# z430/keyword-spotting

Measured on AMD Instinct MI355X. Metric: 1s 16kHz clips/sec end-to-end (wav->label), higher is better.
Workload: dtype f32

## Files before the change

keyword-spotting_amd/csrc/kws_dscnn.hip:

```cpp
#include <array>
#include <utility>

#include "kws_dscnn_stages.h"

namespace kws {
namespace {

#ifndef KWS_X_DSCNN_STAMP_TID
#define KWS_X_DSCNN_STAMP_TID 0
#endif

__device__ __forceinline__ DscnnWeights weights_for_this_clip() {
#if defined(__HIP_DEVICE_COMPILE__)
    using KArg = const __attribute__((address_space(4))) DscnnWeights*;
    KArg p = (KArg)__builtin_amdgcn_kernarg_segment_ptr();
    asm volatile("" : "+s"(p));
    return *p;
#else
    return DscnnWeights{};
#endif
}

using FwdKernelFn = void (*)(DscnnWeights, const float*, int, float*, int32_t*, float*, unsigned long long*, const int*, StreamPush);
struct FwdKernelArgs {
// ... 3 lines not shown
    float* logits;
    int32_t* label;
    float* act;
    unsigned long long* stamps;
    const int* ring_hops;
    StreamPush sp;
};

__device__ __forceinline__ ScanWindows scan_windows_now() {
#if defined(__HIP_DEVICE_COMPILE__)
    using KArg = const __attribute__((address_space(4))) FwdKernelArgs*;
    KArg p = (KArg)__builtin_amdgcn_kernarg_segment_ptr();
    asm volatile("" : "+s"(p));
    return p->sp.scan;
#else
    return ScanWindows{};
#endif
}

template <bool SCAN>
__device__ __forceinline__ const float* clip_features(const float* __restrict__ feat, int clip, const ScanWindows& sw) {
    if constexpr (SCAN) {
        unsigned rec = __umulhi((unsigned)clip, sw.wpr_recip), win = (unsigned)clip - rec * sw.wpr;
        if (win >= sw.wpr) {
            win -= sw.wpr;
            ++rec;
        }
        return feat + (size_t)rec * sw.row_floats + (size_t)win * sw.win_floats;
    } else {
        return feat + (size_t)clip * (IN_T * IN_F);
    }
}

template <bool PAIR, bool SCAN = false>
__device__ __forceinline__ void stage_features_persist(float* lds, const float* __restrict__ feat, int clip, int tid,
                                                       const ScanWindows& sw = ScanWindows{}) {
    constexpr int ST = STAGE_WAVES * 64;
    constexpr int FV = (IN_T * IN_F + ST - 1) / ST;
    static_assert(2 * STAGE_WAVES == NW, "each staging wavefront zeroes the maximum slot of one other wavefront");
    const int lane = tid & 63, wv = tid >> 6;
    const float* f = clip_features<SCAN>(feat, clip, sw);
    float fv[FV];
#pragma unroll
    for (int k = 0; k < FV; ++k) {
        const int i = tid + k * ST;
        fv[k] = i < IN_T * IN_F ? f[i] : 0.f;
    }
    float* featp = lds + OFF_FEAT_P;
    for (int i = tid; i < FEAT_H * FEAT_W; i += ST) {
        const int r = i / FEAT_W - 2, c = i % FEAT_W - 2;
        if (!((unsigned)r < (unsigned)IN_T && (unsigned)c < (unsigned)IN_F)) featp[i] = 0.f;
    }
#pragma unroll
    for (int k = 0; k < FV; ++k) {
        const int i = tid + k * ST;
        if (i < IN_T * IN_F) featp[(i / IN_F + 2) * FEAT_W + (i % IN_F) + 2] = fv[k];
    }
    if constexpr (PAIR) {
        float m = 0.f;
#pragma unroll
        for (int k = 0; k < FV; ++k) m = fmaxf(m, fabsf(fv[k]));
        publish_wave_max(lds, 0, wv, lane, m);
        if (lane == 63) lds[OFF_WMAX + wv + STAGE_WAVES] = 0.f;
    }
}

__device__ __forceinline__ void pool_fc_wave(const DscnnWeights& w, const float* lds, int lane, int clip, float* __restrict__ logits,
                                             int32_t* __restrict__ label, float* __restrict__ a_pool) {
    const int C = w.num_classes;
    float4 fcw[CH / 4];
    float fcb = 0.f;
    const float4* wr = reinterpret_cast<const float4*>(w.fc_w + (lane < C ? lane : 0) * CH);
#pragma unroll
    for (int c = 0; c < CH / 4; ++c) fcw[c] = wr[c];
    if (lane < C) fcb = w.fc_b[lane];
    const float ring_b = w.pw_b[3 * CH + lane];
    constexpr float RING_N = 55.f * 11.f - 53.f * 9.f;
    float s = 0.f;
#pragma unroll
    for (int k = 0; k < NW; ++k) s += lds[OFF_POOLBUF_P + k * CH + lane];
    s = fmaf(RING_N, relu(ring_b), s) * (1.0f / (55.f * 11.f));
    if (a_pool) a_pool[lane] = s;
    float acc = fcb;
#pragma unroll
    for (int c = 0; c < CH / 4; ++c) {
        const float4 a4 = fcw[c];
        acc = fmaf(a4.x, __builtin_bit_cast(float, __builtin_amdgcn_readlane(__builtin_bit_cast(int, s), 4 * c + 0)), acc);
        acc = fmaf(a4.y, __builtin_bit_cast(float, __builtin_amdgcn_readlane(__builtin_bit_cast(int, s), 4 * c + 1)), acc);
        acc = fmaf(a4.z, __builtin_bit_cast(float, __builtin_amdgcn_readlane(__builtin_bit_cast(int, s), 4 * c + 2)), acc);
        acc = fmaf(a4.w, __builtin_bit_cast(float, __builtin_amdgcn_readlane(__builtin_bit_cast(int, s), 4 * c + 3)), acc);
    }
    if (lane < C) logits[(size_t)clip * C + lane] = acc;
    const int idx = wave_argmax_first(lane < C ? acc : -INFINITY, lane, C);
    if (label && lane == 0) label[clip] = idx;
}

// ... 5 lines not shown
                                                           unsigned long long* __restrict__ stamps_arg,
                                                           const int* __restrict__ ring_hops, StreamPush sp) {
    static_assert(!STREAM || (MODE >= 4 && !DIAG && !PRECONV), "the fused push exists for the product paths only");
    static_assert(!PERSIST || ((MODE == 4 || MODE == 5) && !PRECONV && !STREAM), "persistent workgroups: batched product paths only");
    static_assert(!SCAN || ((MODE == 4 || MODE == 5) && !DIAG && !PRECONV && !STREAM && !CLUSTER), "strided windows: batched product paths only");
    constexpr bool PAIR = MODE == 5;
    constexpr int NP = PAIR ? 2 : 3;
    BlockTables t1_pre{};
    static_assert(!CLUSTER || STREAM, "time-tile clusters exist for the streaming push only");
    float* const act = DIAG ? act_arg : nullptr;
    unsigned long long* const stamps = DIAG ? stamps_arg : nullptr;
    extern __shared__ __attribute__((aligned(16))) float lds[];
    constexpr bool MFMA = MODE != 0;
    const int tid_k = threadIdx.x;
    const int lane_k = tid_k & 63, wv_k = tid_k >> 6;

    const int cl_n = CLUSTER ? sp.cluster : 1;
    int clip = CLUSTER ? (int)blockIdx.x / cl_n : (int)blockIdx.x;
    const int cl_tile = CLUSTER ? (int)blockIdx.x - clip * cl_n : 0;
    if (clip >= B) return;
    const int j0 = Blk<4>::H * cl_tile / cl_n, j1 = Blk<4>::H * (cl_tile + 1) / cl_n;
    auto rows = [&](int lo, int hi, int H, int W) { return PosRange{(lo < 0 ? 0 : lo) * W, (hi > H ? H : hi) * W}; };
    const PosRange rg4 = rows(j0, j1, Blk<4>::H, Blk<4>::W), rg3 = rows(j0 - 2, j1, Blk<3>::H, Blk<3>::W),
                   rg2 = rows(j0 - 4, j1, Blk<2>::H, Blk<2>::W), rg1 = rows(j0 - 6, j1, Blk<1>::H, Blk<1>::W),
                   rg0 = rows(j0 - 7, j1 + 1, C1_H, C1_W);
    int n_stamp = 0;
    auto stamp = [&]() {
        if (stamps && tid_k == KWS_X_DSCNN_STAMP_TID) stamps[(size_t)clip * KWS_DSCNN_STAMPS + n_stamp] = __builtin_amdgcn_s_memtime();
        ++n_stamp;
    };

    constexpr bool SPLIT = MODE >= 4;
    constexpr bool UT = PERSIST && PAIR;
    BlockTables t1p{};
    uintx4 c1p[PERSIST ? 7 : 1][NP];
    int prev_clip = -1;
    float* a_prev = nullptr;
    if ((MODE == 4 || MODE == 5) && !CLUSTER && tid_k == 0) lds[OFF_ARRIVE] = 0.f;
    if constexpr (PERSIST) {
        fetch_block_tables(w_arg, 1, tid_k, t1p);
        if (wv_k < STAGE_WAVES) stage_features_persist<PAIR, SCAN>(lds, feat, clip, tid_k, sp.scan);
        load_conv1_frags(w_arg, wv_k, lane_k, c1p);
        __syncthreads();
    }
    for (;;) {
    auto weights_now = [&]() -> DscnnWeights { return PERSIST ? weights_for_this_clip() : w_arg; };
    const DscnnWeights w = weights_now();
    int tid = tid_k;
    if constexpr (PERSIST) {
        int wv_l = __builtin_amdgcn_readfirstlane(wv_k), lane_l = lane_k;
        asm volatile("" : "+s"(wv_l), "+v"(lane_l));
        tid = (wv_l << 6) | (lane_l & 63);
    }
    const int lane = tid & 63, wv = tid >> 6;
    if constexpr (PERSIST) n_stamp = 0;
    if (stamps && tid == KWS_X_DSCNN_STAMP_TID) stamps[(size_t)clip * KWS_DSCNN_STAMPS + KWS_DSCNN_STAMPS - 2] = __builtin_amdgcn_s_memrealtime();
    stamp();

    PwOperands<MODE> wa;
    UnitDesc ud{};
    int hops_before = 0;
    int kx = 0, ky[5] = {0, 0, 0, 0, 0}, sg[5] = {0, 0, 0, 0, 0};
    if constexpr (PERSIST) {
        if constexpr (PAIR) {
            const float mxf = read_stage_max(lds, 0, 1);
            kx = pow2_exp_for(mxf);
            const float bz0 = (w.c1_abs * mxf + w.c1_bmax) * 1.001f;
            cap_units(kx, sg[0], w.k_c1, bz0);
            const float by1 = (w.dw_abs[0] * bz0 + w.dw_bmax[0]) * 1.001f;
            ky[1] = pow2_exp_for(by1);
            cap_units(ky[1], sg[1], w.k_pw[0], (w.pw_abs[0] * by1 + w.pw_bmax[0]) * 1.001f);
            store_block_tables(lds, 1, tid, t1p, pow2f(ky[1]), pow2f(sg[1]), pow2f(ky[1] - sg[0]));
            conv1_build_windows(lds, tid, pow2f(kx), OFF_FEAT_P);
            __syncthreads();
        } else {
            store_block_tables(lds, 1, tid, t1p);
        }
        stamp();
        conv1_phase_split<false, NP>(w, lds, tid, c1p, rg0, pow2f(kx), pow2f(sg[0]), OFF_FEAT_P);
        if (wv == NW - 1 && prev_clip >= 0) {
            pool_fc_wave(w, lds, lane, prev_clip, logits, label, a_prev);
            if (stamps && lane == 0) stamps[(size_t)prev_clip * KWS_DSCNN_STAMPS + 13] = __builtin_amdgcn_s_memtime();
        }
        if constexpr (UT) load_unit_desc(w, 1, wv < Leftover<1>::TILE ? wv : Leftover<1>::TILE, lane, ud);
        load_afrag(w, 1, wv >= 4 ? wv - 4 : 0, lane, wa.ring[0]);
    } else if constexpr (PRECONV) {
        static_assert(!PRECONV || MODE >= 4, "the pre-convolved entry exists for the product (split) path only");
        const float* z = feat + (size_t)clip * (CH * P0);
        fetch_block_tables(w, 1, tid, t1_pre);
        float zmax = 0.f;
        for (int i = tid; i < CH * P0; i += NT) {
            const float v = z[i];
            lds[OFF_Z0 + pidx(i / P0, i % P0, P0 + 2)] = v;
            zmax = fmaxf(zmax, v);
        }
        if (tid < CH) {
            lds[OFF_Z0 + pidx(tid, P0, P0 + 2)] = 0.f;
            lds[OFF_Z0 + pidx(tid, P0 + 1, P0 + 2)] = 0.f;
        }
        if constexpr (PAIR)
            publish_wave_max(lds, 1, wv, lane, zmax);
        else
            store_block_tables(lds, 1, tid, t1_pre);
        if constexpr (Leftover<1>::HAS && (MODE == 4 || MODE == 5) && !CLUSTER)
            load_afrag(w, 1, wv >= 4 ? wv - 4 : 0, lane, wa.ring[0]);
        else
            load_block_head(w, 1, lane, wa);
        stamp();
    } else {
    float* featp = lds + OFF_FEAT;
    const float* f = clip_features<SCAN>(feat, clip, sp.scan);
    constexpr int FV = (IN_T * IN_F + NT - 1) / NT;
// ... 95 lines not shown
    } else {
        conv1_phase<MFMA>(w, lds, tid, a1);
    }
    }
    stamp();
    const DscnnWeights w1 = weights_now();
    __syncthreads();
    stamp();
    float* a = act ? act + (size_t)clip * KWS_ACT_FLOATS_PER_CLIP : nullptr;
    if (a) {
        const float u = PAIR ? pow2f(-sg[0]) : 1.f;
        for (int i = tid; i < CH * P0; i += NT) a[i] = lds[OFF_Z0 + pidx(i / P0, i % P0, P0 + 2)] * u;
        a += CH * P0;
    }
    PairCtx pc;
    if constexpr (PAIR && PRECONV) {
        const float mz0 = read_stage_max(lds, 1, 1);
        const float by1 = (w1.dw_abs[0] * mz0 + w1.dw_bmax[0]) * 1.001f;
        ky[1] = pow2_exp_for(by1);
        cap_units(ky[1], sg[1], w1.k_pw[0], (w1.pw_abs[0] * by1 + w1.pw_bmax[0]) * 1.001f);
        store_block_tables(lds, 1, tid, t1_pre, pow2f(ky[1]), pow2f(sg[1]), pow2f(ky[1]));
        __syncthreads();
    }
    if constexpr (PAIR) {
        const float mz = read_stage_max(lds, 1, 1) * pow2f(-sg[0]);
        const float bz = (w1.pw_abs[0] * ((w1.dw_abs[0] * mz + w1.dw_bmax[0]) * 1.001f) + w1.pw_bmax[0]) * 1.001f;
        const float by = (w1.dw_abs[1] * bz + w1.dw_bmax[1]) * 1.001f;
        ky[2] = pow2_exp_for(by);
        cap_units(ky[2], sg[2], w1.k_pw[1], (w1.pw_abs[1] * by + w1.pw_bmax[1]) * 1.001f);
        pc.s_dww = pow2f(ky[2] - sg[1]);
        pc.s_dwb = pow2f(ky[2]);
        pc.s_pwb = pow2f(sg[2]);
    }
    block_phase<1, MODE, CLUSTER, UT>(w1, lds, tid, wa, ud, nullptr, rg1, pc);
    stamp();
    const DscnnWeights w2 = weights_now();
    __syncthreads();
    stamp();
    if (a) {
        const float u = PAIR ? pow2f(-sg[1]) : 1.f;
        for (int i = tid; i < CH * Blk<1>::POUT; i += NT)
            a[i] = lds[OFF_Z1 + pidx(i / Blk<1>::POUT, i % Blk<1>::POUT, Blk<1>::SOUT)] * u;
        a += CH * Blk<1>::POUT;
    }
    if constexpr (PAIR) {
        const float mz = fmaxf(read_stage_max(lds, 2, 1) * pow2f(-sg[1]), w2.pw_bmax[0]);
        const float bz = (w2.pw_abs[1] * ((w2.dw_abs[1] * mz + w2.dw_bmax[1]) * 1.001f) + w2.pw_bmax[1]) * 1.001f;
        const float by = (w2.dw_abs[2] * bz + w2.dw_bmax[2]) * 1.001f;
        ky[3] = pow2_exp_for(by);
        cap_units(ky[3], sg[3], w2.k_pw[2], (w2.pw_abs[2] * by + w2.pw_bmax[2]) * 1.001f);
        pc.s_dww = pow2f(ky[3] - sg[2]);
        pc.s_dwb = pow2f(ky[3]);
        pc.s_pwb = pow2f(sg[3]);
    }
    block_phase<2, MODE, CLUSTER, UT>(w2, lds, tid, wa, ud, nullptr, rg2, pc);
    stamp();
    const DscnnWeights w3 = weights_now();
    __syncthreads();
    stamp();
    if (a) {
        const float u = PAIR ? pow2f(-sg[2]) : 1.f;
        for (int i = tid; i < CH * Blk<2>::POUT; i += NT)
            a[i] = lds[OFF_Z2 + pidx(i / Blk<2>::POUT, i % Blk<2>::POUT, Blk<2>::SOUT)] * u;
        a += CH * Blk<2>::POUT;
    }
    if constexpr (PAIR) {
        const float mz = fmaxf(read_stage_max(lds, 0, 1) * pow2f(-sg[2]), w3.pw_bmax[1]);
        const float bz = (w3.pw_abs[2] * ((w3.dw_abs[2] * mz + w3.dw_bmax[2]) * 1.001f) + w3.pw_bmax[2]) * 1.001f;
        const float by = (w3.dw_abs[3] * bz + w3.dw_bmax[3]) * 1.001f;
        ky[4] = pow2_exp_for(by);
        cap_units(ky[4], sg[4], w3.k_pw[3], (w3.pw_abs[3] * by + w3.pw_bmax[3]) * 1.001f);
        pc.s_dww = pow2f(ky[4] - sg[3]);
        pc.s_dwb = pow2f(ky[4]);
        pc.s_pwb = pow2f(sg[4]);
    }
    block_phase<3, MODE, CLUSTER, UT>(w3, lds, tid, wa, ud, nullptr, rg3, pc);
    stamp();
    const DscnnWeights w4 = weights_now();
    __syncthreads();
    stamp();
    if (a) {
        const float u = PAIR ? pow2f(-sg[3]) : 1.f;
        for (int i = tid; i < CH * Blk<3>::POUT; i += NT)
            a[i] = lds[OFF_Z3 + pidx(i / Blk<3>::POUT, i % Blk<3>::POUT, Blk<3>::SOUT)] * u;
        a += CH * Blk<3>::POUT;
    }
    if constexpr (PAIR) {
        pc.inv_out = pow2f(-sg[4]);
    }
    block_phase<4, MODE, CLUSTER, UT>(w4, lds, tid, wa, ud, a ? a + CH : nullptr, rg4, pc,
                                      PERSIST ? OFF_POOLBUF_P : OFF_POOLBUF);
    stamp();
    if constexpr (PERSIST) {
        const int next = clip + (int)gridDim.x;
        __builtin_amdgcn_sched_barrier(0);
        const ScanWindows sw_next = SCAN ? scan_windows_now() : ScanWindows{};
        if (wv < STAGE_WAVES && next < B) stage_features_persist<PAIR, SCAN>(lds, feat, next, tid, sw_next);
        stamp();
        load_conv1_frags(w4, wv, lane, c1p);
        __syncthreads();
        stamp();
        if (stamps && tid == KWS_X_DSCNN_STAMP_TID) stamps[(size_t)clip * KWS_DSCNN_STAMPS + KWS_DSCNN_STAMPS - 1] = __builtin_amdgcn_s_memrealtime();
        prev_clip = clip;
        a_prev = a;
        clip = next;
        if (clip >= B) break;
        continue;
    }
    const int C = w4.num_classes;
    float4 fcw[CH / 4];
    float fcb = 0.f, ring_b = 0.f;
    if (wv == 0 && lane < C) {
        const float4* wr = reinterpret_cast<const float4*>(w4.fc_w + lane * CH);
#pragma unroll
        for (int c = 0; c < CH / 4; ++c) fcw[c] = wr[c];
        fcb = w4.fc_b[lane];
    }
    if (tid < CH) ring_b = w4.pw_b[3 * CH + tid];
    __syncthreads();
    stamp();

    float* pooled = lds + OFF_POOLED;
    constexpr float RING_N = 55.f * 11.f - 53.f * 9.f;
    bool run_fc = true;
    if constexpr (CLUSTER) {
        float* part = sp.cl_part + ((size_t)clip * cl_n + cl_tile) * CH;
        if (tid < CH) {
            float s = 0.f;
#pragma unroll
            for (int k = 0; k < NW; ++k) s += lds[OFF_POOLBUF + k * CH + tid];
// ... 182 lines not shown
```

keyword-spotting_amd/csrc/kws_dscnn_geom.h:

```cpp
#pragma once
#include "kws_internal.h"

namespace kws {
namespace {

#ifndef KWS_DSCNN_WAVES
#define KWS_DSCNN_WAVES 8
#endif
constexpr int NW = KWS_DSCNN_WAVES;
constexpr int NT = NW * 64;
constexpr int TW = 30;

constexpr int P0 = C1_H * C1_W;
constexpr int FEAT_H = 103, FEAT_W = 14;
constexpr int OFF_Z3 = 0, OFF_Z2 = 22976, OFF_Z1 = 0, OFF_Z0 = 9152, OFF_FEAT = 18304;
constexpr int OFF_DWTAB = 38784;
constexpr int OFF_PWB = OFF_DWTAB + 2 * 768;
constexpr int OFF_POOLED = OFF_PWB + 2 * 64;
constexpr int OFF_POOLBUF = OFF_DWTAB;
constexpr int OFF_WMAX = OFF_POOLED + 64 + 8;
constexpr int OFF_ARRIVE = OFF_WMAX + 3 * NW;
constexpr int LDS_FLOATS = 40960;
static_assert(OFF_ARRIVE + 1 <= LDS_FLOATS, "LDS overflow");
static_assert(NW * 64 <= 768, "pool scratch must fit one depthwise buffer");
static_assert(OFF_FEAT + FEAT_H * FEAT_W <= OFF_Z2, "feature pad overlaps Z2");
static_assert(CH * 12 <= 2 * NT, "table staging assumes at most two elements per thread");

__host__ __device__ __forceinline__ constexpr int pidx(int c, int p, int S) { return (c >> 1) * 2 * S + 2 * p + (c & 1); }

template <int N>
struct Blk {
    static constexpr int H = 45 + 2 * N, W = 1 + 2 * N;
    static constexpr bool RING = N > 1;
    static constexpr int HI = RING ? H - 2 : H, WI = RING ? W - 2 : W;
    static constexpr int PIN = HI * WI, SIN = PIN + 2;
    static constexpr int POUT = H * W, SOUT = POUT + 2;
    static constexpr int OFF_IN = N == 1 ? OFF_Z0 : N == 2 ? OFF_Z1 : N == 3 ? OFF_Z2 : OFF_Z3;
    static constexpr int OFF_OUT = N == 1 ? OFF_Z1 : N == 2 ? OFF_Z2 : OFF_Z3;
    static constexpr int TILES = (POUT + TW - 1) / TW;
    static constexpr int BUF = (N - 1) & 1;
};

#ifndef KWS_DSCNN_KSPLIT_LEFTOVER
#define KWS_DSCNN_KSPLIT_LEFTOVER 1
#endif
template <int N>
struct Leftover {
    static constexpr bool HAS = KWS_DSCNN_KSPLIT_LEFTOVER && (N == 1 || N == 2);
    static constexpr int TILE = N == 1 ? 4 : 8;
    static constexpr int P0T = TILE * TW;
    static constexpr int NP = HAS ? Blk<N>::POUT - P0T : 1;
    static constexpr int WAVE0 = N == 1 ? 4 : 0;
    static constexpr int OFF_PART = N == 1 ? OFF_Z2 : OFF_Z0;
    static constexpr int CSTRIDE = CH + 4;
    static constexpr int PART = NP * CSTRIDE;
};
static_assert(Blk<1>::TILES == 5 && Blk<2>::TILES == 9, "the leftover tiles are the fifth of block 1 and the ninth of block 2");
static_assert(4 * Leftover<1>::PART <= 38784 - OFF_Z2 && OFF_Z0 + 4 * Leftover<2>::PART <= OFF_FEAT, "partial sums fit their dead planes");
static_assert(Leftover<1>::OFF_PART % 4 == 0 && Leftover<2>::OFF_PART % 4 == 0 && Leftover<1>::CSTRIDE % 4 == 0, "partial sums move as float4s");

constexpr int OFF_FEAT_P = OFF_Z2;
constexpr int OFF_POOLBUF_P = OFF_FEAT_P + 1456;
constexpr int STAGE_WAVES = 4;
static_assert(OFF_FEAT_P >= OFF_Z3 + Blk<3>::SOUT * CH, "the next clip's features must not overlap block 4's input");
static_assert(OFF_FEAT_P + FEAT_H * FEAT_W <= OFF_POOLBUF_P && OFF_POOLBUF_P % 4 == 0, "features and pool partials are disjoint");
static_assert(OFF_POOLBUF_P + NW * CH <= OFF_Z2 + Blk<2>::SOUT * CH && OFF_Z2 + Blk<2>::SOUT * CH <= OFF_DWTAB,
              "pool partials stay inside the Z2 plane, clear of the table buffers the next clip's block 1 rewrites");

}
}
```

keyword-spotting_amd/csrc/kws_dscnn_stages.h:

```cpp
#pragma once
#include <type_traits>

#include "kws_dscnn_geom.h"
#include "kws_dscnn_units.h"
#include "kws_mfcc_dev.h"
#include "kws_split_mfma.h"

namespace kws {
namespace {

template <bool TO_MFMA = false>
__device__ __forceinline__ float stencil3x3(float w0, float w1, float w2, float w3, float w4, float w5, float w6,
                                            float w7, float w8, float b, float up, float mid, float dn, float mask_l,
                                            float mask_r) {
    float c, to_right, to_left;
    asm("v_mul_f32 %1, %3, %13\n\t"
        "v_mul_f32 %2, %5, %13\n\t"
        "v_fma_f32 %0, %4, %13, %12\n\t"
        "v_fmac_f32 %1, %6, %14\n\t"
        "v_fmac_f32 %2, %8, %14\n\t"
        "v_fmac_f32 %0, %7, %14\n\t"
        "v_fmac_f32 %1, %9, %15\n\t"
        "v_fmac_f32 %2, %11, %15\n\t"
        "v_fmac_f32 %0, %10, %15\n\t"
// ... 272 lines not shown
            if (kb + 3 < 7) gather(kb + 3, y[nxt]);
            __builtin_amdgcn_sched_barrier(0);
            product(5);
        }
        if (DUAL && kb + 2 < 7) {
            load_other(kb + 2);
            __builtin_amdgcn_sched_barrier(0);
        }
    }
    acc += acc2;
    occ += occ2;
    if (pos < p_hi) {
#pragma unroll
        for (int r = 0; r < 16; r += 2) {
            const int co = ct * 32 + row_of(r, half);
            const float v0 = relu(fmaf(w.c1_b[co], sig0, acc[r])), v1 = relu(fmaf(w.c1_b[co + 1], sig0, acc[r + 1]));
            *reinterpret_cast<float2*>(z0 + pidx(co, pos, P0 + 2)) = make_float2(v0, v1);
            if constexpr (PAIR) mx = fmaxf(mx, fmaxf(v0, v1));
            if (DUAL) {
                const int oo = (ct ^ 1) * 32 + row_of(r, half);
                const float u0 = relu(fmaf(w.c1_b[oo], sig0, occ[r])), u1 = relu(fmaf(w.c1_b[oo + 1], sig0, occ[r + 1]));
                *reinterpret_cast<float2*>(z0 + pidx(oo, pos, P0 + 2)) = make_float2(u0, u1);
                if constexpr (PAIR) mx = fmaxf(mx, fmaxf(u0, u1));
            }
        }
    }
}

constexpr int C1W_ROWS = FEAT_H;
constexpr int OFF_C1W8 = OFF_Z1;
constexpr int OFF_C1P2 = OFF_C1W8 + 2 * C1W_ROWS * 3 * 4;
static_assert(OFF_C1P2 + 2 * C1W_ROWS * 3 <= OFF_Z0, "conv1's operand windows live where block 1's output goes later");
static_assert(2 * (C1_W - 1) + 9 < FEAT_W && 2 * (C1_H - 1) + 9 < FEAT_H, "window reach inside the padded map");

__device__ __forceinline__ void conv1_build_windows(float* lds, int tid, float sx, int off_feat = OFF_FEAT) {
    const float* featp = lds + off_feat;
    uint32_t* w8 = reinterpret_cast<uint32_t*>(lds + OFF_C1W8);
    uint32_t* p2 = reinterpret_cast<uint32_t*>(lds + OFF_C1P2);
    for (int i = tid; i < C1W_ROWS * 3; i += NT) {
        const float* src = featp + (i / 3) * FEAT_W + 2 * (i % 3);
        const float y[8] = {src[0], src[1], src[2], src[3], src[4], src[5], src[6], src[7]};
        uintx4 hi, lo;
        split_pair8(y, sx, hi, lo);
        *reinterpret_cast<uintx4*>(w8 + i * 4) = hi;
        *reinterpret_cast<uintx4*>(w8 + (C1W_ROWS * 3 + i) * 4) = lo;
        uint32_t h, l;
        split_pair2(src[8], src[9], sx, h, l);
        p2[i] = h;
        p2[C1W_ROWS * 3 + i] = l;
    }
}

template <bool DUAL>
__device__ __forceinline__ void conv1_unit_pairwin(const DscnnWeights& w, const float* lds, float* z0, int ptile, int ct, int lane,
                                                   const uintx4 (&c1f)[7][2], int p_lo, int p_hi, float sig0, float& mx) {
    const int half = lane >> 5, col = lane & 31;
    const int pos = p_lo + ptile * 32 + col;
    const int posc = pos < p_hi ? pos : p_hi - 1;
    const int oh = posc / C1_W, ow = posc % C1_W;
    const int wi = (2 * oh + 5 * half) * 3 + ow;
    const uintx4* w8 = reinterpret_cast<const uintx4*>(lds + OFF_C1W8) + wi;
    const uint32_t* p2 = reinterpret_cast<const uint32_t*>(lds + OFF_C1P2) + wi;
    const floatx16 zero = {0, 0, 0, 0, 0, 0, 0, 0, 0, 0, 0, 0, 0, 0, 0, 0};
    floatx16 acc = zero, acc2 = zero, occ = zero, occ2 = zero;
    const uintx4* osrc = reinterpret_cast<const uintx4*>(w.c1_pair) + (size_t)(ct ^ 1) * (7 * 2 * 64) + lane;
    uintx4 of[DUAL ? 7 : 1][2];
    if (DUAL) {
#pragma unroll
        for (int kb = 0; kb < 7; ++kb) {
            of[kb][0] = osrc[(kb * 2 + 0) * 64];
            of[kb][1] = osrc[(kb * 2 + 1) * 64];
        }
    }
    float4 cb[4], ob[DUAL ? 4 : 1];
#pragma unroll
    for (int q = 0; q < 4; ++q) {
        cb[q] = *reinterpret_cast<const float4*>(w.c1_b + ct * 32 + 8 * q + 4 * half);
        if (DUAL) ob[DUAL ? q : 0] = *reinterpret_cast<const float4*>(w.c1_b + (ct ^ 1) * 32 + 8 * q + 4 * half);
    }
    uintx4 bq[3][2];
    auto b_load = [&](int kb, uintx4 (&d)[2]) {
        if (kb < 5) {
            d[0] = w8[kb * 3];
            d[1] = w8[kb * 3 + C1W_ROWS * 3];
        } else if (kb == 5) {
#pragma unroll
            for (int i = 0; i < 4; ++i) {
                d[0][i] = p2[i * 3];
                d[1][i] = p2[i * 3 + C1W_ROWS * 3];
            }
        } else {
            d[0] = uintx4{p2[4 * 3], 0u, 0u, 0u};
            d[1] = uintx4{p2[4 * 3 + C1W_ROWS * 3], 0u, 0u, 0u};
        }
    };
// ... 7 lines not shown
        if (DUAL) occ2 = mfma_f16(of[DUAL ? kb : 0][0], bl, occ2);
        acc = mfma_f16(c1f[kb][1], bh, acc);
        if (DUAL) occ = mfma_f16(of[DUAL ? kb : 0][1], bh, occ);
        acc2 = mfma_f16(c1f[kb][0], bh, acc2);
        if (DUAL) occ2 = mfma_f16(of[DUAL ? kb : 0][0], bh, occ2);
    }
    acc += acc2;
    occ += occ2;
    if (pos < p_hi) {
#pragma unroll
        for (int r = 0; r < 16; r += 2) {
            const int co = ct * 32 + row_of(r, half);
            const float4 b4 = cb[r >> 2];
            const float b0 = (r & 2) ? b4.z : b4.x, b1 = (r & 2) ? b4.w : b4.y;
            const float v0 = relu(fmaf(b0, sig0, acc[r])), v1 = relu(fmaf(b1, sig0, acc[r + 1]));
            *reinterpret_cast<float2*>(z0 + pidx(co, pos, P0 + 2)) = make_float2(v0, v1);
            mx = fmaxf(mx, fmaxf(v0, v1));
            if (DUAL) {
                const int oo = (ct ^ 1) * 32 + row_of(r, half);
                const float4 o4 = ob[DUAL ? (r >> 2) : 0];
                const float c0 = (r & 2) ? o4.z : o4.x, c1 = (r & 2) ? o4.w : o4.y;
                const float u0 = relu(fmaf(c0, sig0, occ[r])), u1 = relu(fmaf(c1, sig0, occ[r + 1]));
                *reinterpret_cast<float2*>(z0 + pidx(oo, pos, P0 + 2)) = make_float2(u0, u1);
                mx = fmaxf(mx, fmaxf(u0, u1));
            }
        }
    }
}

struct PosRange {
    int lo, hi;
};

template <bool RANGED, int NP>
__device__ __forceinline__ void conv1_phase_split(const DscnnWeights& w, float* lds, int tid, const uintx4 (&c1f)[7][NP],
                                                  PosRange rg, float sx = 1.f, float sig0 = 1.f, int off_feat = OFF_FEAT) {
    static_assert(P0 > 4 * 32 && P0 <= 5 * 32 && NW >= 6, "conv1 work split: four dual tiles + one tile in two halves");
    const float* featp = lds + off_feat;
    float* z0 = lds + OFF_Z0;
    const int lane = tid & 63, wv = tid >> 6;
    float mx = 0.f;
    if constexpr (NP == 2) {
        if constexpr (RANGED) {
            const int n_pt = (rg.hi - rg.lo + 31) / 32;
            for (int u = wv; u < 2 * n_pt; u += NW) conv1_unit_pairwin<false>(w, lds, z0, u >> 1, u & 1, lane, c1f, rg.lo, rg.hi, sig0, mx);
        } else if (wv < 4)
            conv1_unit_pairwin<true>(w, lds, z0, wv, wv & 1, lane, c1f, 0, P0, sig0, mx);
        else if (wv < 6)
            conv1_unit_pairwin<false>(w, lds, z0, 4, wv & 1, lane, c1f, 0, P0, sig0, mx);
    } else if constexpr (RANGED) {
        const int n_pt = (rg.hi - rg.lo + 31) / 32;
        for (int u = wv; u < 2 * n_pt; u += NW) conv1_unit_split<false, NP>(w, featp, z0, u >> 1, u & 1, lane, c1f, rg.lo, rg.hi, sx, sig0, mx);
    } else if (wv < 4)
        conv1_unit_split<true, NP>(w, featp, z0, wv, wv & 1, lane, c1f, 0, P0, sx, sig0, mx);
    else if (wv < 6)
        conv1_unit_split<false, NP>(w, featp, z0, 4, wv & 1, lane, c1f, 0, P0, sx, sig0, mx);
    if constexpr (NP == 2) publish_wave_max(lds, 1, wv, lane, mx);
    if (tid < CH) {
        z0[pidx(tid, P0, P0 + 2)] = 0.f;
        z0[pidx(tid, P0 + 1, P0 + 2)] = 0.f;
    }
}

template <int N, int NP, bool UT = false>
__device__ __forceinline__ void leftover_partial_unit(float* lds, int lane, int M, const uintx4 (&af)[2][NP], const UnitDesc& ud) {
    using G = Blk<N>;
    using L = Leftover<N>;
    const int half = lane >> 5, col = lane & 31;
    const float* dwtab = lds + OFF_DWTAB + G::BUF * 768;
    const float4* dwt4 = reinterpret_cast<const float4*>(dwtab) + half * 24;
    bool valid;
    float mask_l, mask_r;
    int ta[3];
    if constexpr (UT) {
        valid = ud.a[3] != 0u;
        mask_l = __builtin_bit_cast(float, ud.m.x), mask_r = __builtin_bit_cast(float, ud.m.y);
#pragma unroll
        for (int i = 0; i < 3; ++i) ta[i] = (int)ud.a[i];
    } else {
        const int pos = L::P0T - 1 + col;
        valid = col >= 1 && col <= TW && pos < G::POUT;
        const int posc = pos < G::POUT ? pos : G::POUT - 1;
// ... 71 lines not shown
        const int cq = lane & 15;
        const float4 b = reinterpret_cast<const float4*>(lds + OFF_PWB + G::BUF * 64)[cq];
        constexpr int ROUNDS = (L::NP + 3) / 4, RB = 2;
        static_assert(ROUNDS % RB == 0, "whole batches");
        auto comb = [&](float p0, float p1, float p2, float p3, float bias) { return relu(((p0 + p1) + (p2 + p3)) + bias); };
#pragma unroll 1
        for (int r0 = 0; r0 < ROUNDS; r0 += RB) {
            float4 p[RB][4];
#pragma unroll
            for (int r = 0; r < RB; ++r) {
                const int j = (lane >> 4) + 4 * (r0 + r);
                const int jc = j < L::NP ? j : L::NP - 1;
#pragma unroll
                for (int m = 0; m < 4; ++m) p[r][m] = part4[(m * L::PART + jc * L::CSTRIDE) / 4 + cq];
            }
#pragma unroll
            for (int r = 0; r < RB; ++r) {
                const int j = (lane >> 4) + 4 * (r0 + r);
                const float4(&q)[4] = p[r];
                const float v0 = comb(q[0].x, q[1].x, q[2].x, q[3].x, b.x), v1 = comb(q[0].y, q[1].y, q[2].y, q[3].y, b.y);
                const float v2 = comb(q[0].z, q[1].z, q[2].z, q[3].z, b.z), v3 = comb(q[0].w, q[1].w, q[2].w, q[3].w, b.w);
                if (j < L::NP) {
                    *reinterpret_cast<float2*>(zout + pidx(4 * cq, L::P0T + j, G::SOUT)) = make_float2(v0, v1);
                    *reinterpret_cast<float2*>(zout + pidx(4 * cq + 2, L::P0T + j, G::SOUT)) = make_float2(v2, v3);
                    mx = fmaxf(mx, fmaxf(fmaxf(v0, v1), fmaxf(v2, v3)));
                }
            }
        }
        if (lane == 0) *arrived = 0;
    }
    return mx;
}

template <int N, int MODE, bool RANGED = false, bool UT = false>
__device__ __forceinline__ void block_phase(const DscnnWeights& w, float* lds, int tid, PwOperands<MODE>& pwo, UnitDesc& ud,
                                            float* __restrict__ act4 = nullptr, PosRange rg = PosRange{0, 0}, PairCtx pc = PairCtx{},
                                            int off_poolbuf = OFF_POOLBUF) {
    static_assert(!UT || ((MODE == 4 || MODE == 5) && !RANGED && Leftover<1>::HAS), "unit descriptors: product paths on whole maps");
    using G = Blk<N>;
    constexpr bool PAIR = MODE == 5;
    constexpr int NP = PAIR ? 2 : 3;
    constexpr int NPROD = PAIR ? 3 : 6;
    constexpr bool KSL = Leftover<N>::HAS && (MODE == 4 || MODE == 5) && !RANGED;
    const int p_lo = RANGED ? rg.lo : 0, p_hi = RANGED ? rg.hi : G::POUT;
#ifdef KWS_X_DSCNN_SKIP_LEFTOVER
    const int n_tiles = RANGED ? (p_hi - p_lo + TW - 1) / TW : (N == 2 ? 8 : G::TILES);
#else
    const int n_tiles = RANGED ? (p_hi - p_lo + TW - 1) / TW : (KSL ? Leftover<N>::TILE : G::TILES);
#endif
    constexpr bool MFMA = MODE != 0;
    constexpr bool SPLIT = MODE >= 4;
    constexpr bool NO_STENCIL = MODE == 6;
    const int lane = tid & 63, wv = tid >> 6, half = lane >> 5, col = lane & 31;
    float* zout = lds + G::OFF_OUT;
    const float* dwtab = lds + OFF_DWTAB + G::BUF * 768;
    const float* pwb = lds + OFF_PWB + G::BUF * 64;
    float* poolbuf = lds + off_poolbuf;

    BlockTables next_tables;
    if constexpr (N < 4) {
        fetch_block_tables(w, N + 1, tid, next_tables);
        if (tid < CH) {
            zout[pidx(tid, G::POUT, G::SOUT)] = relu(pwb[tid]);
            zout[pidx(tid, G::POUT + 1, G::SOUT)] = 0.f;
        }
    } else if (!MFMA) {
        poolbuf[wv * CH + lane] = 0.f;
    }

    const float4* bias4 = reinterpret_cast<const float4*>(pwb) + half;
    const float4* dwt4 = reinterpret_cast<const float4*>(dwtab) + half * 24;
    float psum[2][16];
#pragma unroll
    for (int ct = 0; ct < 2; ++ct)
#pragma unroll
        for (int r = 0; r < 16; ++r) psum[ct][r] = 0.f;
    float stage_max = 0.f;

    for (int t = wv; t < n_tiles; t += NW) {
        const int pos = p_lo + t * TW - 1 + col;
        bool valid;
        uint32_t keep;
        float mask_l, mask_r;
        int tlo[3], thi[3];
        if constexpr (UT) {
            keep = ud.a[3];
            valid = keep != 0u;
            mask_l = __builtin_bit_cast(float, ud.m.x), mask_r = __builtin_bit_cast(float, ud.m.y);
#pragma unroll
            for (int i = 0; i < 3; ++i) {
                tlo[i] = (int)ud.a[i];
                thi[i] = tlo[i] + 32 * G::SIN;
                asm volatile("" : "+v"(tlo[i]));
                asm volatile("" : "+v"(thi[i]));
            }
        } else {
            valid = col >= 1 && col <= TW && pos < p_hi;
            keep = valid ? 0xffffffffu : 0u;
            const int posc = pos < p_lo ? p_lo : (pos < p_hi ? pos : p_hi - 1);
            const int h = posc / G::W, x = posc % G::W;
            mask_l = x > 0 ? 1.f : 0.f, mask_r = x < G::W - 1 ? 1.f : 0.f;
#pragma unroll
            for (int dh = -1; dh <= 1; ++dh) {
                const int o = G::RING ? 1 : 0;
                const int hh = h + dh - o, xx = x - o;
                const bool inside = (unsigned)hh < (unsigned)G::HI && (unsigned)xx < (unsigned)G::WI;
                const bool in_map = (unsigned)(h + dh) < (unsigned)G::H;
                const int a = inside ? hh * G::WI + xx : ((G::RING && in_map) ? G::PIN : G::PIN + 1);
                tlo[dh + 1] = G::OFF_IN + pidx(half * 8, a, G::SIN);
                thi[dh + 1] = tlo[dh + 1] + 32 * G::SIN;
                asm volatile("" : "+v"(tlo[dh + 1]));
// ... 56 lines not shown
                            acc1 = mfma_f16(pwo.ring[m & 1][1][pa], b, acc1);
                    } else {
                        if (ct == 0)
                            acc0 = mfma_bf16(pwo.ring[m & 1][0][pa], b, acc0);
                        else
                            acc1 = mfma_bf16(pwo.ring[m & 1][1][pa], b, acc1);
                    }
                    __builtin_amdgcn_sched_barrier(0);
                };
#pragma unroll
                for (int s = 0; s < 32; ++s) {
                    const int m = s >> 3, j = s & 7;
                    DwPair& wp = (s & 2) ? wq1 : wq0;
                    TapPair& tq = (s & 2) ? tq1 : tq0;
                    const bool feed = m > 0 && j < NPROD;
                    if (feed) product(0, m - 1, j);
                    if constexpr (NO_STENCIL)
                        y[j] = (s & 1) ? tq.mid.y : tq.mid.x;
                    else
                        y[j] = (s & 1) ? dw_eval(wp, tq, std::integral_constant<int, 1>{}) : dw_eval(wp, tq, std::integral_constant<int, 0>{});
                    __builtin_amdgcn_sched_barrier(0);
                    if (feed) product(1, m - 1, j);
                    if ((s & 1) && s + 3 < 32) {
                        if constexpr (!NO_STENCIL) wts_pair_load((s >> 1) + 2, wp);
                        tap_pair_load((s >> 1) + 2, tq);
                    }
                    __builtin_amdgcn_sched_barrier(0);
                    if (j == 6) {
                        if (m < 3) {
                            load_afrag(w, N, m + 1, lane, pwo.ring[(m + 1) & 1]);
                        } else if (t + NW < n_tiles) {
                            if constexpr (UT) load_unit_desc(w, N, t + NW, lane, ud_next);
                            load_afrag(w, N, 0, lane, pwo.ring[0]);
                        } else if (KSL && N == 2 && wv < 4) {
                            if constexpr (UT) load_unit_desc(w, N, Leftover<N>::TILE, lane, ud_next);
                            load_afrag(w, N, wv, lane, pwo.ring[0]);
                        } else if (N < 4) {
                            if constexpr (UT) load_unit_desc(w, N < 4 ? N + 1 : N, wv, lane, ud_next);
                            load_afrag(w, N < 4 ? N + 1 : N, 0, lane, pwo.ring[0]);
                        }
                        __builtin_amdgcn_sched_barrier(0);
                    }
                    if (j == 7) {
                        if constexpr (PAIR) {
                            split_pair8_scaled(y, bh, bl);
                        } else {
                            split3(y, bh, bm, bl);
                        }
                        __builtin_amdgcn_sched_barrier(0);
                    }
                }
#pragma unroll
                for (int q = 0; q < NPROD; ++q) {
                    product(0, 3, q);
                    product(1, 3, q);
                }
            } else {
                auto& wa = pwo.wa;
#pragma unroll
                for (int s = 0; s < 32; s += 2) {
                    TapPair& tq = (s & 2) ? tq1 : tq0;
                    DwPair& wp = (s & 2) ? wq1 : wq0;
                    float y0, y1;
                    if constexpr (MODE == 2) {
                        y0 = tq.mid.x;
                        y1 = tq.mid.y;
                    } else {
                        y0 = dw_eval(wp, tq, std::integral_constant<int, 0>{});
                        y1 = dw_eval(wp, tq, std::integral_constant<int, 1>{});
// ... 71 lines not shown
            epilogue();
            if constexpr (UT) ud = ud_next;
        } else {
            const float* pw_w = w.pw_w + (N - 1) * CH * CH;
            float y[32];
#pragma unroll
            for (int s = 0; s < 32; s += 2) {
                TapPair tq;
                tap_pair_load(s >> 1, tq);
                DwPair wp;
                wts_pair_load(s >> 1, wp);
                y[s] = dw_eval(wp, tq, std::integral_constant<int, 0>{});
                y[s + 1] = dw_eval(wp, tq, std::integral_constant<int, 1>{});
            }
#pragma unroll 1
            for (int co = 0; co < CH; ++co) {
                float part = 0.f;
#pragma unroll
                for (int s = 0; s < 32; ++s) part = fmaf(pw_w[(16 * (s >> 3) + 8 * half + (s & 7)) * CH + co], y[s], part);
                const float tot = relu(part + __shfl_xor(part, 32, 64) + pwb[co]);
                if constexpr (N < 4) {
                    if (valid && half == 0) zout[pidx(co, pos, G::SOUT)] = tot;
                } else {
                    if (act4 && valid && half == 0) act4[co * G::POUT + pos] = tot;
                    float sum = (valid && half == 0) ? tot : 0.f;
#pragma unroll
                    for (int o = 16; o >= 1; o >>= 1) sum += __shfl_xor(sum, o, 64);
                    if (lane == 0) poolbuf[wv * CH + co] += sum;
                }
            }
        }
    }

    if constexpr (KSL) {
        using L = Leftover<N>;
        if (wv >= L::WAVE0 && wv < L::WAVE0 + 4) {
            leftover_partial_unit<N, NP, UT>(lds, lane, wv - L::WAVE0, pwo.ring[0], ud);
            __builtin_amdgcn_sched_barrier(0);
            if constexpr (UT) load_unit_desc(w, N + 1, wv, lane, ud);
            load_afrag(w, N + 1, 0, lane, pwo.ring[0]);
            __builtin_amdgcn_sched_barrier(0);
            stage_max = fmaxf(stage_max, leftover_arrive<N>(lds, lane));
        }
    }
    if constexpr (N < 4) store_block_tables(lds, N + 1, tid, next_tables, pc.s_dwb, pc.s_pwb, pc.s_dww);
    if constexpr (PAIR && N <= 2) publish_wave_max(lds, N == 1 ? 2 : 0, wv, lane, stage_max);
    if constexpr (MFMA) {
        if constexpr (N < 4) {
            if (wv >= n_tiles && !(KSL && N == 1)) load_block_head(w, N + 1, lane, pwo);
        } else {
#pragma unroll
            for (int ct = 0; ct < 2; ++ct) {
                float (&q)[16] = psum[ct];
                asm volatile("s_nop 4\n\t"
                    "v_add_f32_dpp %0, %0, %0 row_shr:1 row_mask:0xf bank_mask:0xf bound_ctrl:1\n\t"
                    "v_add_f32_dpp %1, %1, %1 row_shr:1 row_mask:0xf bank_mask:0xf bound_ctrl:1\n\t"
                    "v_add_f32_dpp %2, %2, %2 row_shr:1 row_mask:0xf bank_mask:0xf bound_ctrl:1\n\t"
                    "v_add_f32_dpp %3, %3, %3 row_shr:1 row_mask:0xf bank_mask:0xf bound_ctrl:1\n\t"
                    "v_add_f32_dpp %4, %4, %4 row_shr:1 row_mask:0xf bank_mask:0xf bound_ctrl:1\n\t"
                    "v_add_f32_dpp %5, %5, %5 row_shr:1 row_mask:0xf bank_mask:0xf bound_ctrl:1\n\t"
                    "v_add_f32_dpp %6, %6, %6 row_shr:1 row_mask:0xf bank_mask:0xf bound_ctrl:1\n\t"
                    "v_add_f32_dpp %7, %7, %7 row_shr:1 row_mask:0xf bank_mask:0xf bound_ctrl:1\n\t"
                    "v_add_f32_dpp %8, %8, %8 row_shr:1 row_mask:0xf bank_mask:0xf bound_ctrl:1\n\t"
                    "v_add_f32_dpp %9, %9, %9 row_shr:1 row_mask:0xf bank_mask:0xf bound_ctrl:1\n\t"
                    "v_add_f32_dpp %10, %10, %10 row_shr:1 row_mask:0xf bank_mask:0xf bound_ctrl:1\n\t"
                    "v_add_f32_dpp %11, %11, %11 row_shr:1 row_mask:0xf bank_mask:0xf bound_ctrl:1\n\t"
                    "v_add_f32_dpp %12, %12, %12 row_shr:1 row_mask:0xf bank_mask:0xf bound_ctrl:1\n\t"
// ... 103 lines not shown
```

Before: 7.490 million.

## Build next clip's conv1 windows in last staging wave; run block-2 leftover quarter first

```diff
diff --git a/keyword-spotting_amd/csrc/kws_dscnn.hip b/keyword-spotting_amd/csrc/kws_dscnn.hip
--- a/keyword-spotting_amd/csrc/kws_dscnn.hip
+++ b/keyword-spotting_amd/csrc/kws_dscnn.hip
@@ -59,8 +59,9 @@
     }
 }
 
-template <bool PAIR, bool SCAN = false>
-__device__ __forceinline__ void stage_features_persist(float* lds, const float* __restrict__ feat, int clip, int tid,
+constexpr bool TAIL_WINDOWS = KWS_DSCNN_TAIL_WINDOWS;
+template <bool PAIR, bool SCAN = false, typename WeightsNow>
+__device__ __forceinline__ void stage_features_persist(float* lds, const float* __restrict__ feat, int clip, int tid, WeightsNow weights_now,
                                                        const ScanWindows& sw = ScanWindows{}) {
     constexpr int ST = STAGE_WAVES * 64;
     constexpr int FV = (IN_T * IN_F + ST - 1) / ST;
@@ -89,6 +90,25 @@
         for (int k = 0; k < FV; ++k) m = fmaxf(m, fabsf(fv[k]));
         publish_wave_max(lds, 0, wv, lane, m);
         if (lane == 63) lds[OFF_WMAX + wv + STAGE_WAVES] = 0.f;
+        if constexpr (TAIL_WINDOWS) {
+            int* staged = reinterpret_cast<int*>(lds + OFF_STAGED);
+            asm volatile("s_waitcnt lgkmcnt(0)" ::: "memory");
+            int before = 0;
+            if (lane == 0) before = __hip_atomic_fetch_add(staged, 1, __ATOMIC_RELAXED, __HIP_MEMORY_SCOPE_WORKGROUP);
+            before = __builtin_amdgcn_readfirstlane(before);
+            asm volatile("" ::: "memory");
+            if (before == STAGE_WAVES - 1) {
+                C1WindowSrc src;
+                conv1_windows_wave_read(lds, lane, OFF_FEAT_P, src);
+                const float mxf = read_stage_max(lds, 0, 1);
+                const DscnnWeights w = weights_now();
+                __builtin_amdgcn_sched_barrier(0);
+                int kx = pow2_exp_for(mxf), sg0;
+                cap_units(kx, sg0, w.k_c1, (w.c1_abs * mxf + w.c1_bmax) * 1.001f);
+                conv1_windows_wave_store<OFF_C1WIN_P>(lds, lane, pow2f(kx), src);
+                if (lane == 0) *staged = 0;
+            }
+        }
     }
 }
 
@@ -160,14 +180,21 @@
 
     constexpr bool SPLIT = MODE >= 4;
     constexpr bool UT = PERSIST && PAIR;
+    constexpr bool QF = PERSIST && (KWS_DSCNN_QUARTER_FIRST == 2 || (KWS_DSCNN_QUARTER_FIRST == 1 && !PAIR));
     BlockTables t1p{};
     uintx4 c1p[PERSIST ? 7 : 1][NP];
     int prev_clip = -1;
     float* a_prev = nullptr;
     if ((MODE == 4 || MODE == 5) && !CLUSTER && tid_k == 0) lds[OFF_ARRIVE] = 0.f;
+    constexpr bool TAILWIN = PERSIST && PAIR && TAIL_WINDOWS;
+    constexpr int OFF_WIN = TAILWIN ? OFF_C1WIN_P : OFF_C1W8;
     if constexpr (PERSIST) {
         fetch_block_tables(w_arg, 1, tid_k, t1p);
-        if (wv_k < STAGE_WAVES) stage_features_persist<PAIR, SCAN>(lds, feat, clip, tid_k, sp.scan);
+        if constexpr (TAILWIN) {
+            if (tid_k == 0) lds[OFF_STAGED] = 0.f;
+            __syncthreads();
+        }
+        if (wv_k < STAGE_WAVES) stage_features_persist<PAIR, SCAN>(lds, feat, clip, tid_k, [&]() -> const DscnnWeights& { return w_arg; }, sp.scan);
         load_conv1_frags(w_arg, wv_k, lane_k, c1p);
         __syncthreads();
     }
@@ -199,13 +226,16 @@
             ky[1] = pow2_exp_for(by1);
             cap_units(ky[1], sg[1], w.k_pw[0], (w.pw_abs[0] * by1 + w.pw_bmax[0]) * 1.001f);
             store_block_tables(lds, 1, tid, t1p, pow2f(ky[1]), pow2f(sg[1]), pow2f(ky[1] - sg[0]));
-            conv1_build_windows(lds, tid, pow2f(kx), OFF_FEAT_P);
-            __syncthreads();
+            if constexpr (TAILWIN) {
+            } else {
+                conv1_build_windows(lds, tid, pow2f(kx), OFF_FEAT_P);
+                __syncthreads();
+            }
         } else {
             store_block_tables(lds, 1, tid, t1p);
         }
         stamp();
-        conv1_phase_split<false, NP>(w, lds, tid, c1p, rg0, pow2f(kx), pow2f(sg[0]), OFF_FEAT_P);
+        conv1_phase_split<false, NP, OFF_WIN>(w, lds, tid, c1p, rg0, pow2f(kx), pow2f(sg[0]), OFF_FEAT_P);
         if (wv == NW - 1 && prev_clip >= 0) {
             pool_fc_wave(w, lds, lane, prev_clip, logits, label, a_prev);
             if (stamps && lane == 0) stamps[(size_t)prev_clip * KWS_DSCNN_STAMPS + 13] = __builtin_amdgcn_s_memtime();
@@ -367,7 +397,7 @@
         pc.s_dwb = pow2f(ky[2]);
         pc.s_pwb = pow2f(sg[2]);
     }
-    block_phase<1, MODE, CLUSTER, UT>(w1, lds, tid, wa, ud, nullptr, rg1, pc);
+    block_phase<1, MODE, CLUSTER, UT, QF>(w1, lds, tid, wa, ud, nullptr, rg1, pc);
     stamp();
     const DscnnWeights w2 = weights_now();
     __syncthreads();
@@ -388,7 +418,7 @@
         pc.s_dwb = pow2f(ky[3]);
         pc.s_pwb = pow2f(sg[3]);
     }
-    block_phase<2, MODE, CLUSTER, UT>(w2, lds, tid, wa, ud, nullptr, rg2, pc);
+    block_phase<2, MODE, CLUSTER, UT, QF>(w2, lds, tid, wa, ud, nullptr, rg2, pc);
     stamp();
     const DscnnWeights w3 = weights_now();
     __syncthreads();
@@ -430,7 +460,7 @@
         const int next = clip + (int)gridDim.x;
         __builtin_amdgcn_sched_barrier(0);
         const ScanWindows sw_next = SCAN ? scan_windows_now() : ScanWindows{};
-        if (wv < STAGE_WAVES && next < B) stage_features_persist<PAIR, SCAN>(lds, feat, next, tid, sw_next);
+        if (wv < STAGE_WAVES && next < B) stage_features_persist<PAIR, SCAN>(lds, feat, next, tid, weights_now, sw_next);
         stamp();
         load_conv1_frags(w4, wv, lane, c1p);
         __syncthreads();
diff --git a/keyword-spotting_amd/csrc/kws_dscnn_geom.h b/keyword-spotting_amd/csrc/kws_dscnn_geom.h
--- a/keyword-spotting_amd/csrc/kws_dscnn_geom.h
+++ b/keyword-spotting_amd/csrc/kws_dscnn_geom.h
@@ -20,8 +20,9 @@
 constexpr int OFF_POOLBUF = OFF_DWTAB;
 constexpr int OFF_WMAX = OFF_POOLED + 64 + 8;
 constexpr int OFF_ARRIVE = OFF_WMAX + 3 * NW;
+constexpr int OFF_STAGED = OFF_ARRIVE + 1;
 constexpr int LDS_FLOATS = 40960;
-static_assert(OFF_ARRIVE + 1 <= LDS_FLOATS, "LDS overflow");
+static_assert(OFF_STAGED + 1 <= LDS_FLOATS, "LDS overflow");
 static_assert(NW * 64 <= 768, "pool scratch must fit one depthwise buffer");
 static_assert(OFF_FEAT + FEAT_H * FEAT_W <= OFF_Z2, "feature pad overlaps Z2");
 static_assert(CH * 12 <= 2 * NT, "table staging assumes at most two elements per thread");
@@ -43,6 +44,9 @@
 
 #ifndef KWS_DSCNN_KSPLIT_LEFTOVER
 #define KWS_DSCNN_KSPLIT_LEFTOVER 1
+#endif
+#ifndef KWS_DSCNN_QUARTER_FIRST
+#define KWS_DSCNN_QUARTER_FIRST 1
 #endif
 template <int N>
 struct Leftover {
@@ -66,6 +70,15 @@
 static_assert(OFF_FEAT_P + FEAT_H * FEAT_W <= OFF_POOLBUF_P && OFF_POOLBUF_P % 4 == 0, "features and pool partials are disjoint");
 static_assert(OFF_POOLBUF_P + NW * CH <= OFF_Z2 + Blk<2>::SOUT * CH && OFF_Z2 + Blk<2>::SOUT * CH <= OFF_DWTAB,
               "pool partials stay inside the Z2 plane, clear of the table buffers the next clip's block 1 rewrites");
+#ifndef KWS_DSCNN_TAIL_WINDOWS
+#define KWS_DSCNN_TAIL_WINDOWS 1
+#endif
+constexpr int C1WIN_DWORDS = 2 * FEAT_H * 3 * 4 + 2 * FEAT_H * 3;
+constexpr int OFF_C1WIN_P = OFF_POOLBUF_P + NW * CH;
+static_assert(OFF_C1WIN_P % 4 == 0 && OFF_C1WIN_P >= OFF_Z3 + Blk<3>::SOUT * CH && OFF_C1WIN_P + C1WIN_DWORDS <= OFF_Z2 + Blk<2>::SOUT * CH,
+              "the next clip's windows: 16-byte aligned, behind the pool partials, inside the Z2 plane (dead from block 3's barrier), clear of block 4's input");
+static_assert(Leftover<1>::OFF_PART == OFF_Z2 && Leftover<2>::OFF_PART + 4 * Leftover<2>::PART <= OFF_Z2,
+              "of the leftover partials only block 1's overwrite the windows: behind conv1's barrier, when the windows are dead");
 
 }
 }
diff --git a/keyword-spotting_amd/csrc/kws_dscnn_stages.h b/keyword-spotting_amd/csrc/kws_dscnn_stages.h
--- a/keyword-spotting_amd/csrc/kws_dscnn_stages.h
+++ b/keyword-spotting_amd/csrc/kws_dscnn_stages.h
@@ -328,6 +328,7 @@
 constexpr int OFF_C1P2 = OFF_C1W8 + 2 * C1W_ROWS * 3 * 4;
 static_assert(OFF_C1P2 + 2 * C1W_ROWS * 3 <= OFF_Z0, "conv1's operand windows live where block 1's output goes later");
 static_assert(2 * (C1_W - 1) + 9 < FEAT_W && 2 * (C1_H - 1) + 9 < FEAT_H, "window reach inside the padded map");
+static_assert(OFF_C1P2 + 2 * C1W_ROWS * 3 - OFF_C1W8 == C1WIN_DWORDS, "the windows' size as kws_dscnn_geom.h places it");
 
 __device__ __forceinline__ void conv1_build_windows(float* lds, int tid, float sx, int off_feat = OFF_FEAT) {
     const float* featp = lds + off_feat;
@@ -347,7 +348,43 @@
     }
 }
 
-template <bool DUAL>
+struct C1WindowSrc {
+    static constexpr int ITEMS = C1W_ROWS * 3, ROUNDS = (ITEMS + 63) / 64;
+    float2 y[ROUNDS][5];
+};
+__device__ __forceinline__ void conv1_windows_wave_read(const float* lds, int lane, int off_feat, C1WindowSrc& s) {
+    static_assert(FEAT_W % 2 == 0 && OFF_FEAT % 2 == 0 && OFF_FEAT_P % 2 == 0, "a window starts at an even column: 8-byte reads");
+#pragma unroll
+    for (int r = 0; r < C1WindowSrc::ROUNDS; ++r) {
+        const int i = lane + 64 * r;
+        const int ic = i < C1WindowSrc::ITEMS ? i : C1WindowSrc::ITEMS - 1;
+        const float2* src = reinterpret_cast<const float2*>(lds + off_feat + (ic / 3) * FEAT_W + 2 * (ic % 3));
+#pragma unroll
+        for (int k = 0; k < 5; ++k) s.y[r][k] = src[k];
+    }
+}
+template <int OFF_WIN>
+__device__ __forceinline__ void conv1_windows_wave_store(float* lds, int lane, float sx, const C1WindowSrc& s) {
+    uint32_t* w8 = reinterpret_cast<uint32_t*>(lds + OFF_WIN);
+    uint32_t* p2 = reinterpret_cast<uint32_t*>(lds + OFF_WIN + (OFF_C1P2 - OFF_C1W8));
+#pragma unroll
+    for (int r = 0; r < C1WindowSrc::ROUNDS; ++r) {
+        const int i = lane + 64 * r;
+        const float y[8] = {s.y[r][0].x, s.y[r][0].y, s.y[r][1].x, s.y[r][1].y, s.y[r][2].x, s.y[r][2].y, s.y[r][3].x, s.y[r][3].y};
+        uintx4 hi, lo;
+        split_pair8(y, sx, hi, lo);
+        uint32_t h, l;
+        split_pair2(s.y[r][4].x, s.y[r][4].y, sx, h, l);
+        if (i < C1WindowSrc::ITEMS) {
+            *reinterpret_cast<uintx4*>(w8 + i * 4) = hi;
+            *reinterpret_cast<uintx4*>(w8 + (C1W_ROWS * 3 + i) * 4) = lo;
+            p2[i] = h;
+            p2[C1W_ROWS * 3 + i] = l;
+        }
+    }
+}
+
+template <bool DUAL, int OFF_WIN = OFF_C1W8>
 __device__ __forceinline__ void conv1_unit_pairwin(const DscnnWeights& w, const float* lds, float* z0, int ptile, int ct, int lane,
                                                    const uintx4 (&c1f)[7][2], int p_lo, int p_hi, float sig0, float& mx) {
     const int half = lane >> 5, col = lane & 31;
@@ -355,8 +392,8 @@
     const int posc = pos < p_hi ? pos : p_hi - 1;
     const int oh = posc / C1_W, ow = posc % C1_W;
     const int wi = (2 * oh + 5 * half) * 3 + ow;
-    const uintx4* w8 = reinterpret_cast<const uintx4*>(lds + OFF_C1W8) + wi;
-    const uint32_t* p2 = reinterpret_cast<const uint32_t*>(lds + OFF_C1P2) + wi;
+    const uintx4* w8 = reinterpret_cast<const uintx4*>(lds + OFF_WIN) + wi;
+    const uint32_t* p2 = reinterpret_cast<const uint32_t*>(lds + OFF_WIN + (OFF_C1P2 - OFF_C1W8)) + wi;
     const floatx16 zero = {0, 0, 0, 0, 0, 0, 0, 0, 0, 0, 0, 0, 0, 0, 0, 0};
     floatx16 acc = zero, acc2 = zero, occ = zero, occ2 = zero;
     const uintx4* osrc = reinterpret_cast<const uintx4*>(w.c1_pair) + (size_t)(ct ^ 1) * (7 * 2 * 64) + lane;
@@ -430,7 +467,7 @@
     int lo, hi;
 };
 
-template <bool RANGED, int NP>
+template <bool RANGED, int NP, int OFF_WIN = OFF_C1W8>
 __device__ __forceinline__ void conv1_phase_split(const DscnnWeights& w, float* lds, int tid, const uintx4 (&c1f)[7][NP],
                                                   PosRange rg, float sx = 1.f, float sig0 = 1.f, int off_feat = OFF_FEAT) {
     static_assert(P0 > 4 * 32 && P0 <= 5 * 32 && NW >= 6, "conv1 work split: four dual tiles + one tile in two halves");
@@ -441,11 +478,11 @@
     if constexpr (NP == 2) {
         if constexpr (RANGED) {
             const int n_pt = (rg.hi - rg.lo + 31) / 32;
-            for (int u = wv; u < 2 * n_pt; u += NW) conv1_unit_pairwin<false>(w, lds, z0, u >> 1, u & 1, lane, c1f, rg.lo, rg.hi, sig0, mx);
+            for (int u = wv; u < 2 * n_pt; u += NW) conv1_unit_pairwin<false, OFF_WIN>(w, lds, z0, u >> 1, u & 1, lane, c1f, rg.lo, rg.hi, sig0, mx);
         } else if (wv < 4)
-            conv1_unit_pairwin<true>(w, lds, z0, wv, wv & 1, lane, c1f, 0, P0, sig0, mx);
+            conv1_unit_pairwin<true, OFF_WIN>(w, lds, z0, wv, wv & 1, lane, c1f, 0, P0, sig0, mx);
         else if (wv < 6)
-            conv1_unit_pairwin<false>(w, lds, z0, 4, wv & 1, lane, c1f, 0, P0, sig0, mx);
+            conv1_unit_pairwin<false, OFF_WIN>(w, lds, z0, 4, wv & 1, lane, c1f, 0, P0, sig0, mx);
     } else if constexpr (RANGED) {
         const int n_pt = (rg.hi - rg.lo + 31) / 32;
         for (int u = wv; u < 2 * n_pt; u += NW) conv1_unit_split<false, NP>(w, featp, z0, u >> 1, u & 1, lane, c1f, rg.lo, rg.hi, sx, sig0, mx);
@@ -583,7 +620,7 @@
     return mx;
 }
 
-template <int N, int MODE, bool RANGED = false, bool UT = false>
+template <int N, int MODE, bool RANGED = false, bool UT = false, bool QF = false>
 __device__ __forceinline__ void block_phase(const DscnnWeights& w, float* lds, int tid, PwOperands<MODE>& pwo, UnitDesc& ud,
                                             float* __restrict__ act4 = nullptr, PosRange rg = PosRange{0, 0}, PairCtx pc = PairCtx{},
                                             int off_poolbuf = OFF_POOLBUF) {
@@ -628,6 +665,25 @@
         for (int r = 0; r < 16; ++r) psum[ct][r] = 0.f;
     float stage_max = 0.f;
 
+    constexpr bool QUARTER_FIRST = QF && KSL && N == 2;
+    static_assert(!QF || (Leftover<2>::WAVE0 == 0 && Leftover<1>::TILE == 4), "block 1's tile wavefronts are block 2's quarter wavefronts");
+    if constexpr (QUARTER_FIRST) {
+        if (wv < 4) {
+            UnitDesc ud_q = ud;
+#pragma unroll
+            for (int ct = 0; ct < 2; ++ct)
+#pragma unroll
+                for (int p = 0; p < NP; ++p) pwo.ring[1][ct][p] = pwo.ring[0][ct][p];
+            __builtin_amdgcn_sched_barrier(0);
+            if constexpr (UT) load_unit_desc(w, N, wv, lane, ud);
+            load_afrag(w, N, 0, lane, pwo.ring[0]);
+            __builtin_amdgcn_sched_barrier(0);
+            leftover_partial_unit<N, NP, UT>(lds, lane, wv, pwo.ring[1], ud_q);
+            __builtin_amdgcn_sched_barrier(0);
+            stage_max = fmaxf(stage_max, leftover_arrive<N>(lds, lane));
+        }
+    }
+
     for (int t = wv; t < n_tiles; t += NW) {
         const int pos = p_lo + t * TW - 1 + col;
         bool valid;
@@ -750,9 +806,12 @@
                         } else if (t + NW < n_tiles) {
                             if constexpr (UT) load_unit_desc(w, N, t + NW, lane, ud_next);
                             load_afrag(w, N, 0, lane, pwo.ring[0]);
-                        } else if (KSL && N == 2 && wv < 4) {
+                        } else if (KSL && N == 2 && wv < 4 && !QUARTER_FIRST) {
                             if constexpr (UT) load_unit_desc(w, N, Leftover<N>::TILE, lane, ud_next);
                             load_afrag(w, N, wv, lane, pwo.ring[0]);
+                        } else if (QF && KSL && N == 1) {
+                            if constexpr (UT) load_unit_desc(w, N + 1, Leftover<2>::TILE, lane, ud_next);
+                            load_afrag(w, N + 1, wv, lane, pwo.ring[0]);
                         } else if (N < 4) {
                             if constexpr (UT) load_unit_desc(w, N < 4 ? N + 1 : N, wv, lane, ud_next);
                             load_afrag(w, N < 4 ? N + 1 : N, 0, lane, pwo.ring[0]);
@@ -890,7 +949,7 @@
         }
     }
 
-    if constexpr (KSL) {
+    if constexpr (KSL && !QUARTER_FIRST) {
         using L = Leftover<N>;
         if (wv >= L::WAVE0 && wv < L::WAVE0 + 4) {
             leftover_partial_unit<N, NP, UT>(lds, lane, wv - L::WAVE0, pwo.ring[0], ud);
```

Result: no change. 7.539 million (median of 6 runs) (+0.7%).
